# jeertmans/DiffeRT2d

Hardware: AMD Instinct MI355X
Metric: ray-path candidates/s (higher is better)
Workload: dtype f32

## Files before the change

### differt2d_amd/csrc/d2d_kernels.hpp

```cpp
#pragma once
#include <hip/hip_runtime.h>
#include <stdint.h>

#include "../../include/d2d.h"

namespace d2d {

template <typename T>
__device__ __forceinline__ const __attribute__((address_space(4))) T* cmem(const T* p) {
    return (const __attribute__((address_space(4))) T*)(unsigned long long)p;
}

__device__ __forceinline__ float4 ldc4(const float4* p, long i) {
    typedef float v4f __attribute__((ext_vector_type(4)));
    const v4f v = ((const __attribute__((address_space(4))) v4f*)(unsigned long long)p)[i];
    return make_float4(v.x, v.y, v.z, v.w);
}
__device__ __forceinline__ int4 ldc4i(const int4* p, long i) {
    typedef int v4i __attribute__((ext_vector_type(4)));
    const v4i v = ((const __attribute__((address_space(4))) v4i*)(unsigned long long)p)[i];
    return make_int4(v.x, v.y, v.z, v.w);
}

template <typename T, unsigned OFF>
__device__ __forceinline__ T late_kernarg() {
    static_assert(sizeof(T) == 4 || sizeof(T) == 8, "one or two dwords");
    const auto base = __builtin_amdgcn_kernarg_segment_ptr();
    T v;
    if constexpr (sizeof(T) == 8) asm volatile("s_load_dwordx2 %0, %1, %2\n\ts_waitcnt lgkmcnt(0)" : "=s"(v) : "s"(base), "i"(OFF));
    else asm volatile("s_load_dword %0, %1, %2\n\ts_waitcnt lgkmcnt(0)" : "=s"(v) : "s"(base), "i"(OFF));
    return v;
}
#define D2D_LATE_ARG(T, field) late_kernarg<T, (unsigned)__builtin_offsetof(SweepArgs, field)>()

enum Mode { MODE_HARD = 0, MODE_HSIG = 1, MODE_SIG = 2 };

constexpr int RL_CHUNK = 128;
struct ListPool {
    unsigned long long* pool;
    int* next;
    int* head;
    int n_static;
    int max_chunks;
};
struct RegionLevel {
    int* cnt[D2D_MAX_ORDER + 1];
    int chunk0[D2D_MAX_ORDER + 1];
    int S;
    int R;
    int regions_x, regions_y;
    const float4* box;
    const unsigned long long* hidden;
    float hidden_dperp;
};
struct RegionLists {
    RegionLevel leaf;
    ListPool lp;
    int* flag;
};

struct SweepArgs {
    const RegionLists* __restrict__ rl;
    int* fb_n;
    int* fb_list;
    const float4* __restrict__ occl;
    const float4* __restrict__ refl;
    const float4* __restrict__ flt;
    const int* __restrict__ cw;
    int N, Nc;
    const float* __restrict__ X;
    const float* __restrict__ Y;
    float* __restrict__ out;
    int m, n;
    float txx, txy;
    int min_order, max_order;
    float alpha, tol;
    float seg_lo, seg_hi;
    float flt_lo, flt_hi;
    float on_lo, on_hi;
    float loss_skip;
    float sig_l2f;
    int sig_mono;
    const unsigned long long* __restrict__ shadow;
    float shadow_dperp;
    float shadow_lo, shadow_inv;
    int shadow_prefix_ok;
    const unsigned long long* __restrict__ pair;
    float pair_dperp;
    int pair_prefix_ok;
    float fnum[D2D_MAX_ORDER + 1];
    float h2;
    int fun_id;
    int out_mode;
    float patch;
    float* __restrict__ grad;
    const float* __restrict__ cot;
    float* __restrict__ partial;
    const float* __restrict__ cust_f;
    const float* __restrict__ cust_pb;
    long cust_cells;

    const int* __restrict__ sched;
    int cullq_off;
    int n_heavy;
    int heavy_cap;
    float* __restrict__ heavy_list;
    int* __restrict__ heavy_cnt;
    int* __restrict__ heavy_done;
    unsigned* __restrict__ cost_out;

    unsigned long long* nan_cell_bits;
    unsigned* nan_row_bits;
    int nan_row_words;
    int nan_wqcap, nan_rb;
#ifdef D2D_AB_TIMELINE
    unsigned long long* tl_ring;
    int tl_seq;
#endif
    unsigned long long* stats;
    unsigned long long* wave_cycles;
};

#define D2D_WORK(x) (st.work += (x))
#define D2D_EPS 1.1920929e-07f

struct WaveStats {
    unsigned c[16];
    int shadow;
    unsigned work;
};

__device__ __forceinline__ bool wave_any(bool p) { return __any(p); }

__device__ __forceinline__ int late_index(int i) {
    asm volatile("" : "+s"(i));
    return i;
}

template <int I>
__device__ __forceinline__ void stat_add(WaveStats& st, unsigned long long x) {
    const unsigned x32 = (unsigned)x;
    asm volatile("v_add_u32 %0, %0, %1" : "+v"(st.c[I]) : "v"(x32));
}

#ifndef D2D_FAST_DIV
#define D2D_FAST_DIV 0
#endif
__device__ __forceinline__ bool div_in_range(float x) {
    float ax = fabsf(x);
    return ax >= 2.168404345e-19f && ax <= 4.611686018e18f;
}
__device__ __forceinline__ float rcp_refined(float y) {
    float r = __builtin_amdgcn_rcpf(y);
    float e = __builtin_fmaf(-y, r, 1.0f);
    return __builtin_fmaf(e, r, r);
}
__device__ __forceinline__ float div_with_rcp(float x, float y, float r) {
    float q = x * r;
    float e = __builtin_fmaf(-y, q, x);
    q = __builtin_fmaf(e, r, q);
    e = __builtin_fmaf(-y, q, x);
    return __builtin_fmaf(e, r, q);
}
__device__ __forceinline__ void div2_exact(float x1, float x2, float y, float& q1, float& q2) {
#if D2D_FAST_DIV
    const bool ok = div_in_range(y) && (x1 == 0.0f || div_in_range(x1)) && (x2 == 0.0f || div_in_range(x2));
    if (!wave_any(!ok)) {
        const float r = rcp_refined(y);
        q1 = div_with_rcp(x1, y, r);
        q2 = div_with_rcp(x2, y, r);
        return;
    }
#endif
    q1 = x1 / y;
    q2 = x2 / y;
}
__device__ __forceinline__ float div1_exact(float x, float y) {
#if D2D_FAST_DIV
    const bool ok = div_in_range(y) && (x == 0.0f || div_in_range(x));
    if (!wave_any(!ok)) return div_with_rcp(x, y, rcp_refined(y));
#endif
    return x / y;
}

__device__ __forceinline__ void image_of(const float4& r0, float px, float py, float& ox, float& oy) {
    float ix = px - r0.x, iy = py - r0.y;
    float dn = ix * r0.z + iy * r0.w;
    float s = 2.0f * dn;
    ox = px - s * r0.z;
    oy = py - s * r0.w;
}

__device__ __forceinline__ void normalize2(float vx, float vy, float& ox, float& oy) {
    float len = sqrtf(vx * vx + vy * vy);
    len = (len == 0.0f) ? 1.0f : len;
    ox = vx / len;
    oy = vy / len;
}

template <int B, int E, class F>
__device__ __forceinline__ void static_for(F&& f) {
    if constexpr (B < E) {
        f(std::integral_constant<int, B>{});
        static_for<B + 1, E>(f);
    }
}

__device__ __forceinline__ float clampact(float x, float alpha) {
    float z = alpha * x;
    return fminf(fmaxf(z + 3.0f, 0.0f), 6.0f);
}

static __device__ __constant__ unsigned long long EXPF_TAB[32] = {
    0x3ff0000000000000ull, 0x3fefd9b0d3158574ull, 0x3fefb5586cf9890full, 0x3fef9301d0125b51ull, 0x3fef72b83c7d517bull, 0x3fef54873168b9aaull,
    0x3fef387a6e756238ull, 0x3fef1e9df51fdee1ull, 0x3fef06fe0a31b715ull, 0x3feef1a7373aa9cbull, 0x3feedea64c123422ull, 0x3feece086061892dull,
    0x3feebfdad5362a27ull, 0x3feeb42b569d4f82ull, 0x3feeab07dd485429ull, 0x3feea47eb03a5585ull, 0x3feea09e667f3bcdull, 0x3fee9f75e8ec5f74ull,
    0x3feea11473eb0187ull, 0x3feea589994cce13ull, 0x3feeace5422aa0dbull, 0x3feeb737b0cdc5e5ull, 0x3feec49182a3f090ull, 0x3feed503b23e255dull,
    0x3feee89f995ad3adull, 0x3feeff76f2fb5e47ull, 0x3fef199bdd85529cull, 0x3fef3720dcef9069ull, 0x3fef5818dcfba487ull, 0x3fef7c97337b9b5full,
    0x3fefa4afa2a490daull, 0x3fefd0765b6e4540ull};
__device__ __forceinline__ float expf_libm(float x) {
    if (x != x) return x + x;
    if (x > 0x1.62e42ep6f) return __builtin_inff();
    if (x < -0x1.9fe368p6f) return 0.0f;
    if (x < -0x1.9d1d9ep6f) return 0x1p-149f;
    const double z = (0x1.71547652b82fep+0 * 32.0) * (double)x;
    double kd = z + 0x1.8p+52;
    const unsigned long long ki = (unsigned long long)__double_as_longlong(kd);
    kd = kd - 0x1.8p+52;
    const double r = z - kd;
    const unsigned long long t = EXPF_TAB[ki & 31ull] + (ki << 47);
    const double sc = __longlong_as_double((long long)t);
    const double zz = (0x1.c6af84b912394p-5 / 32.0 / 32.0 / 32.0) * r + (0x1.ebfce50fac4f3p-3 / 32.0 / 32.0);
    const double r2 = r * r;
    double y = (0x1.62e42ff0c52d6p-1 / 32.0) * r + 1.0;
    y = zz * r2 + y;
    y = y * sc;
    return (float)y;
}

__device__ __forceinline__ float sigmoidf_(float z) { return 1.0f / (1.0f + expf_libm(-z)); }

__device__ __forceinline__ float sig_zc_of(float l2f, float acc) {
    const int E = (int)((__float_as_uint(acc) >> 23) & 0xffu) - 127;
    return ((float)(E - 25) - l2f - 0.01f) * 0.69314718f;
}

struct GradCtx {
    float grx, gry;
    float tbx, tby;
    float cot;
    float* wl;
    bool scene;
    int ci;
    long cell;
};

__device__ __forceinline__ float wave_sum(float v) {
#pragma unroll
    for (int off = 32; off > 0; off >>= 1) v += __shfl_xor(v, off, 64);
    return v;
}

template <int MODE>
__device__ __forceinline__ float dact(float x, float alpha) {
    float z = alpha * x;
    if (MODE == MODE_HSIG) {
        float y = z + 3.0f;
        return (y > 0.0f && y < 6.0f) ? alpha / 6.0f : 0.0f;
    }
    float s = sigmoidf_(z);
    return alpha * (s * (1.0f - s));
}

__device__ __forceinline__ void normalize2_bwd(float vx, float vy, float obx, float oby, float& vbx, float& vby) {
    float len = sqrtf(vx * vx + vy * vy);
    bool z = (len == 0.0f);
    len = z ? 1.0f : len;
    float ox = vx / len, oy = vy / len;
    float d = z ? 0.0f : (obx * ox + oby * oy);
    vbx = (obx - d * ox) / len;
    vby = (oby - d * oy) / len;
}

template <int K, int MODE, bool STATS, bool GRAD = false, bool PREF = true, bool TXG = false>
__device__ __forceinline__ void eval_candidate(const SweepArgs& a, const int (&cand)[D2D_MAX_ORDER],
                                               const float (&imgx)[D2D_MAX_ORDER], const float (&imgy)[D2D_MAX_ORDER],
                                               float txx, float txy, float rxx, float rxy, bool lane_bad, float& acc,
                                               WaveStats& st, GradCtx* g = nullptr, float acc_floor = -1.0f) {
    const float zc_acc = (acc_floor >= 0.0f) ? acc_floor : acc;
    int on_i = 0, on_w = 0, hit_i = 0, hit_j = -1;
    float hit2 = -3.0e38f;
    bool znan = false;
    long cust = 0;
    if (GRAD && a.fun_id == D2D_FUN_CUSTOM) cust = (long)(g->ci++) * a.cust_cells + g->cell;
    float px[K + 2], py[K + 2];
    px[0] = txx;
    py[0] = txy;
    px[K + 1] = rxx;
    py[K + 1] = rxy;

    if (PREF && !GRAD && K > 0) {
        const float4 r0 = ldc4(a.refl, 2 * cand[K - 1]);
        const float4 r1 = ldc4(a.refl, 2 * cand[K - 1] + 1);
        const float4 fc = ldc4(a.flt, cand[K - 1]);
        float ux = rxx - imgx[K - 1], uy = rxy - imgy[K - 1];
        float vx = r0.x - rxx, vy = r0.y - rxy;
        float un = ux * r0.z + uy * r0.w;
        float vn = vx * r0.z + vy * r0.w;
        float gq = vn * __builtin_amdgcn_rcpf(un);
        float dx = __builtin_fmaf(gq, ux, -vx), dy = __builtin_fmaf(gq, uy, -vy);
        float sa = __builtin_fmaf(r1.y, dy, r1.x * dx) * fc.x;
        float ex = __builtin_fmaf(fabsf(gq), fabsf(ux), fabsf(vx)) + fabsf(r0.x);
        float ey = __builtin_fmaf(fabsf(gq), fabsf(uy), fabsf(vy)) + fabsf(r0.y);
        float M = __builtin_fmaf(__builtin_fmaf(fabsf(r1.y), ey, fabsf(r1.x) * ex), fc.y, 1e-30f);
        bool cull = !lane_bad && (un != 0.0f) && (ex < 1e18f) && (ey < 1e18f) && ((sa + M < a.on_lo) || (sa - M > a.on_hi));
        if (STATS) stat_add<9>(st, 1);
        if (!wave_any(!cull)) return;
    }

    D2D_WORK(6 + 2 * K);
    if (STATS) {
        stat_add<0>(st, 1);
        stat_add<6>(st, K);
    }
    float sv[K + 1];
    constexpr bool PRE = !GRAD && !TXG && K >= 1;
    unsigned long long sh_pre = 0ull, pm_pre[K + 1];
    constexpr bool HOIST = PRE && K <= 2;
    if (HOIST) {
        if (a.shadow != nullptr) sh_pre = cmem(a.shadow)[cand[0]];
#pragma unroll
        for (int i = 0; i + 1 < K; ++i) pm_pre[i] = (a.pair != nullptr) ? cmem(a.pair)[(size_t)cand[i] * a.N + cand[i + 1]] : 0ull;
    }
    const int sh = (st.shadow >= 0 && st.shadow < a.N) ? st.shadow : -1;
    int j = sh >= 0 ? sh : 0;
    float4 w = ldc4(a.occl, a.N > 0 ? j : 0);
    {
        float ptx = rxx, pty = rxy;
#pragma unroll
        for (int i = K - 1; i >= 0; --i) {
            const float4 r0 = ldc4(a.refl, 2 * cand[i]);
            float ux = ptx - imgx[i], uy = pty - imgy[i];
            float vx = r0.x - ptx, vy = r0.y - pty;
            float un = ux * r0.z + uy * r0.w;
            float vn = vx * r0.z + vy * r0.w;
            bool z = (un == 0.0f);
            float den = z ? 1.0f : un;
            float incx, incy;
            div2_exact(vn * ux, vn * uy, den, incx, incy);
            incx = z ? 0.0f : incx;
            incy = z ? 0.0f : incy;
            ptx = ptx + incx;
            pty = pty + incy;
            px[i + 1] = ptx;
            py[i + 1] = pty;
            if (GRAD && (MODE != MODE_HARD || a.fun_id != D2D_FUN_ONE)) znan = znan || z;
            if (!GRAD) {
                const float4 r1 = ldc4(a.refl, 2 * cand[i] + 1);
                const float dx = ptx - r0.x, dy = pty - r0.y;
                const float sw = div1_exact(r1.x * dx + r1.y * dy, r1.z);
                sv[i] = sw;
                if (i > 0) {
                    bool off;
                    if (MODE == MODE_HARD) off = !((sw >= 0.0f) && (sw <= 1.0f));
                    else if (MODE == MODE_HSIG) off = fminf(clampact(sw - 0.0f, a.alpha), clampact(1.0f - sw, a.alpha)) == 0.0f;
                    else off = fminf(a.alpha * (sw - 0.0f), a.alpha * (1.0f - sw)) <= fmaxf(-89.0f, sig_zc_of(a.sig_l2f, zc_acc));
                    const bool pt_bad = lane_bad || !(fabsf(ptx) < 1e18f) || !(fabsf(pty) < 1e18f);
                    if (!wave_any(!off || pt_bad)) {
                        if (STATS && i == K - 1) stat_add<15>(st, 1);
                        return;
                    }
                }
            }
        }
    }
    if (GRAD && MODE != MODE_HARD && K > 0) {
#pragma unroll
        for (int i = 0; i <= K; ++i) znan = znan || (px[i + 1] == px[i] && py[i + 1] == py[i]);
    }
    if (GRAD && a.fun_id != D2D_FUN_ONE && a.fun_id != D2D_FUN_CUSTOM) {
#pragma unroll
        for (int i = 0; i <= K; ++i) znan = znan || (((px[i + 1] - px[i]) + D2D_EPS == 0.0f) && ((py[i + 1] - py[i]) + D2D_EPS == 0.0f));
    }
    if (GRAD && wave_any(znan)) {
        const float qnan = __builtin_nanf("");
        if (znan) {
            g->grx = qnan;
            g->gry = qnan;
        }
        if (g->scene) {
            if (znan) g->tbx = g->tby = qnan;
            if ((threadIdx.x & 63) == 0) {
#pragma unroll
                for (int i = 0; i < K; ++i) {
                    float* w4 = g->wl + 4 * cand[i];
                    w4[0] = w4[1] = w4[2] = w4[3] = qnan;
                }
            }
        }
    }

    bool bad = lane_bad;
#pragma unroll
    for (int i = 1; i <= K; ++i) bad = bad || !(fabsf(px[i]) < 1e18f) || !(fabsf(py[i]) < 1e18f);
    if (GRAD && a.fun_id == D2D_FUN_CUSTOM) {
        const float* pb = a.cust_pb + cust * (2 * (D2D_MAX_ORDER + 2));
        bad = bad || !(fabsf(a.cust_f[cust]) < 3.0e38f);
#pragma unroll
        for (int i = 0; i < 2 * (K + 2); ++i) bad = bad || !(fabsf(pb[i]) < 3.0e38f);
    }

    bool on_b = true;
    float on_c = 6.0f;
    float on_z = 3.0e38f;
    bool nanflag = false;
#pragma unroll
    for (int i = 0; i < K; ++i) {
        float s;
        if (GRAD) {
            const float4 r0 = ldc4(a.refl, 2 * cand[i]);
            const float4 r1 = ldc4(a.refl, 2 * cand[i] + 1);
            float dx = px[i + 1] - r0.x, dy = py[i + 1] - r0.y;
            s = div1_exact(r1.x * dx + r1.y * dy, r1.z);
            sv[i] = s;
        } else {
            s = sv[i];
        }
        if (MODE == MODE_HARD) {
            on_b = on_b && (s >= 0.0f) && (s <= 1.0f);
        } else if (MODE == MODE_HSIG) {
            nanflag = nanflag || (s != s);
            float c1 = clampact(s - 0.0f, a.alpha), c2 = clampact(1.0f - s, a.alpha);
            float cm = fminf(c1, c2);
            if (GRAD && cm < on_c) {
                on_i = i;
                on_w = (c2 < c1) ? 1 : 0;
            }
            on_c = fminf(on_c, cm);
        } else {
            nanflag = nanflag || (s != s);
            float z1 = a.alpha * (s - 0.0f), z2 = a.alpha * (1.0f - s);
            float zm = fminf(z1, z2);
            if (GRAD && zm < on_z) {
                on_i = i;
                on_w = (z2 < z1) ? 1 : 0;
            }
            on_z = fminf(on_z, zm);
        }
    }
    bool on_zero = (MODE == MODE_HARD) ? !on_b : (MODE == MODE_HSIG) ? (on_c == 0.0f)
                   : (on_z <= (GRAD ? -89.0f : fmaxf(-89.0f, sig_zc_of(a.sig_l2f, zc_acc))));
    if (K > 0 && !wave_any(!on_zero || bad)) return;

    const bool live = !on_zero || bad;
    D2D_WORK(1);

    float bx[K + 1], by[K + 1];
#pragma unroll
    for (int i = 0; i <= K; ++i) {
        bx[i] = px[i] - px[i + 1];
        by[i] = py[i] - py[i + 1];
    }
    bool hit_b = false;
    float hit_c = 0.0f;
    float hit_z = -3.0e38f;
    bool any_test = false;
    bool active = live;
    if (!GRAD && !TXG && K >= 1 && a.shadow != nullptr) {
        const float eps = 1.1920929e-07f;
        bool occl = false;
        float Ei[K + 1];
        float padv[K + 1];
#pragma unroll
        for (int i = 0; i < K; ++i) {
            const float4 r0 = ldc4(a.refl, 2 * cand[i]);
            const float4 r1 = ldc4(a.refl, 2 * cand[i] + 1);
            const float4 fc = ldc4(a.flt, cand[i]);
            const float ex = fabsf(px[i + 1] - px[i + 2]) + fabsf(r0.x - px[i + 2]) + fabsf(r0.x) + fabsf(imgx[i]);
            const float ey = fabsf(py[i + 1] - py[i + 2]) + fabsf(r0.y - py[i + 2]) + fabsf(r0.y) + fabsf(imgy[i]);
            Ei[i] = ex + ey;
            padv[i] = __builtin_fmaf(__builtin_fmaf(fabsf(r1.y), ey, fabsf(r1.x) * ex), fc.y, 1e-4f);
        }
        {
            const unsigned long long shm = HOIST ? sh_pre : cmem(a.shadow)[cand[0]];
            if (shm != 0ull) {
                const float fa_ = (sv[0] - padv[0] - a.shadow_lo) * a.shadow_inv, fb_ = (sv[0] + padv[0] - a.shadow_lo) * a.shadow_inv;
                const bool ok = fa_ >= 0.0f && fb_ < 64.0f && 256.0f * eps * Ei[0] <= a.shadow_dperp;
                const int ka = ok ? (int)fa_ : 0, kb = ok ? (int)fb_ : 0;
                occl = ok && (kb - ka <= 1) && ((shm >> ka) & 1ull) && ((shm >> kb) & 1ull);
            }
        }
        if (K >= 2 && a.pair != nullptr) {
#pragma unroll
            for (int i = 0; i + 1 < K; ++i) {
                const unsigned long long m = HOIST ? pm_pre[i] : cmem(a.pair)[(size_t)cand[i] * a.N + cand[i + 1]];
                if (m != 0ull) {
                    const float k8 = 0.125f * a.shadow_inv;
                    const float ea_ = (sv[i] - padv[i] - a.shadow_lo) * k8, eb_ = (sv[i] + padv[i] - a.shadow_lo) * k8;
                    const float la_ = (sv[i + 1] - padv[i + 1] - a.shadow_lo) * k8, lb_ = (sv[i + 1] + padv[i + 1] - a.shadow_lo) * k8;
                    const bool ok = ea_ >= 0.0f && eb_ < 8.0f && la_ >= 0.0f && lb_ < 8.0f && 512.0f * eps * Ei[i] <= a.pair_dperp &&
                                    512.0f * eps * Ei[i + 1] <= a.pair_dperp;
                    const int ea = ok ? (int)ea_ : 0, eb = ok ? (int)eb_ : 0, la = ok ? (int)la_ : 0, lb = ok ? (int)lb_ : 0;
                    const bool all4 = ((m >> (ea + 8 * la)) & 1ull) && ((m >> (eb + 8 * la)) & 1ull) && ((m >> (ea + 8 * lb)) & 1ull) &&
                                      ((m >> (eb + 8 * lb)) & 1ull);
                    occl = occl || (ok && all4 && (eb - ea <= 1) && (lb - la <= 1));
                }
            }
        }
        if (wave_any(occl)) {
            if (MODE == MODE_HARD) hit_b = hit_b || occl;
            else if (MODE == MODE_HSIG) hit_c = occl ? 6.0f : hit_c;
            else {
                hit_z = occl ? 1.0e30f : hit_z;
                any_test = true;
            }
            active = active && (!occl || bad);
            D2D_WORK(2);
            if (!wave_any(active)) return;
        }
    }
    if (STATS) stat_add<2>(st, 1);
    constexpr bool PAIRS = MODE != MODE_SIG;
    if constexpr (PAIRS) {
    auto filt = [&](const float4& ww, int jj) -> unsigned {
        unsigned wbits = 0u;
#pragma unroll
        for (int i = 0; i <= K; ++i) {
            const int ig0 = (i == 0) ? -1 : cand[i - 1];
            const int ig1 = (i == K) ? -1 : cand[i];
            const bool skip = (jj == ig0 || jj == ig1);
            float Cx = ww.x - px[i], Cy = ww.y - py[i];
            float fa = by[i] * Cx - bx[i] * Cy;
            float fb = ww.z * Cy - ww.w * Cx;
            float fd = ww.w * bx[i] - ww.z * by[i];
            float pa = __builtin_fmaf(-a.flt_lo, fd, fa) * __builtin_fmaf(-a.flt_hi, fd, fa);
            float pb = __builtin_fmaf(-a.flt_lo, fd, fb) * __builtin_fmaf(-a.flt_hi, fd, fb);
            bool miss = fmaxf(pa, pb) > 0.0f;
            if (MODE == MODE_SIG && !skip) any_test = true;
            if (STATS) stat_add<4>(st, skip ? 0 : 1);
            wbits |= (!skip && active && (!miss || bad)) ? (1u << i) : 0u;
        }
        return wbits;
    };
    auto exact = [&](const float4& ww, int jj, unsigned wbits) {
#pragma unroll
        for (int i = 0; i <= K; ++i) {
            if (!wave_any((wbits >> i) & 1u)) continue;
            if (STATS) stat_add<5>(st, 1);
            D2D_WORK(2);
            const float Cx = ww.x - px[i], Cy = ww.y - py[i];
            const float fa = by[i] * Cx - bx[i] * Cy;
            const float fb = ww.z * Cy - ww.w * Cx;
            const float fd = ww.w * bx[i] - ww.z * by[i];
            bool dz = (fd == 0.0f);
            float dd = dz ? 1.0f : fd;
            float ta, tb;
            div2_exact(fa, fb, dd, ta, tb);
            ta = dz ? __builtin_inff() : ta;
            tb = dz ? __builtin_inff() : tb;
            if (MODE == MODE_HARD) {
                bool h = (ta >= a.seg_lo) && (ta <= a.seg_hi) && (tb >= a.seg_lo) && (tb <= a.seg_hi);
                hit_b = hit_b || h;
            } else if (MODE == MODE_HSIG) {
                nanflag = nanflag || (ta != ta) || (tb != tb);
                float c = fminf(fminf(clampact(ta - a.seg_lo, a.alpha), clampact(a.seg_hi - ta, a.alpha)),
                                fminf(clampact(tb - a.seg_lo, a.alpha), clampact(a.seg_hi - tb, a.alpha)));
                if (GRAD && (c > hit_c || (c == hit_c && hit_j >= 0 && (jj < hit_j || (jj == hit_j && i < hit_i))))) {
                    hit_i = i;
                    hit_j = jj;
                }
                if (GRAD) hit2 = (c > hit_c) ? hit_c : fmaxf(hit2, c);
                hit_c = fmaxf(hit_c, c);
            } else {
                nanflag = nanflag || (ta != ta) || (tb != tb);
                float z = fminf(fminf(a.alpha * (ta - a.seg_lo), a.alpha * (a.seg_hi - ta)),
                                fminf(a.alpha * (tb - a.seg_lo), a.alpha * (a.seg_hi - tb)));
                if (GRAD && (z > hit_z || (z == hit_z && hit_j >= 0 && (jj < hit_j || (jj == hit_j && i < hit_i))))) {
                    hit_i = i;
                    hit_j = jj;
                }
                if (GRAD) hit2 = (z > hit_z) ? hit_z : fmaxf(hit2, z);
                hit_z = fmaxf(hit_z, z);
            }
        }
        if (MODE == MODE_HARD) active = active && (!hit_b || bad);
        else if (MODE == MODE_HSIG) active = active && (hit_c != 6.0f || bad);
        else active = active && (hit_z < 17.5f || bad);
    };
    {
        bool done = a.N <= 0;
        if (!done && sh >= 0) {
            const unsigned b0 = filt(w, sh);
            D2D_WORK(K + 1);
            if (wave_any(b0 != 0u)) {
                exact(w, sh, b0);
                if (!wave_any(active)) {
                    st.shadow = sh;
                    done = true;
                }
            }
        }
        auto next_idx = [&](int x) -> int {
            ++x;
            return x == sh ? x + 1 : x;
        };
        int jA = (sh == 0) ? 1 : 0;
        if (!done && jA < a.N) {
            int jB = next_idx(jA);
            float4 wA = (sh >= 0) ? ldc4(a.occl, jA) : w;
            float4 wB = ldc4(a.occl, jB < a.N ? jB : jA);
            while (true) {
                const bool hasB = jB < a.N;
                const int nA = next_idx(jB), nB = next_idx(nA);
                const float4 wnA = ldc4(a.occl, nA < a.N ? nA : jA), wnB = ldc4(a.occl, nB < a.N ? nB : jA);
                const unsigned ba = filt(wA, jA);
                const unsigned bb = hasB ? filt(wB, jB) : 0u;
                D2D_WORK(hasB ? 2 * (K + 1) : (K + 1));
                if (wave_any((ba | bb) != 0u)) {
                    if (wave_any(ba != 0u)) {
                        exact(wA, jA, ba);
                        if (!wave_any(active)) {
                            st.shadow = jA;
                            break;
                        }
                    }
                    if (wave_any(bb != 0u)) {
                        exact(wB, jB, bb);
                        if (!wave_any(active)) {
                            st.shadow = jB;
                            break;
                        }
                    }
                }
                if (!(nA < a.N)) break;
                jA = nA;
                jB = nB;
                wA = wnA;
                wB = wnB;
            }
        }
    }
    } else {
    int nxt = sh >= 0 ? 0 : 1;
    if (nxt == sh) ++nxt;
    for (bool more = a.N > 0; more;) {
        const bool has_next = nxt < a.N;
        const float4 wn = ldc4(a.occl, has_next ? nxt : j);
        float fa_[K + 1], fb_[K + 1], fd_[K + 1];
        unsigned wbits = 0u;
#pragma unroll
        for (int i = 0; i <= K; ++i) {
            const int ig0 = (i == 0) ? -1 : cand[i - 1];
            const int ig1 = (i == K) ? -1 : cand[i];
            const bool skip = (j == ig0 || j == ig1);
            float Cx = w.x - px[i], Cy = w.y - py[i];
            float fa = by[i] * Cx - bx[i] * Cy;
            float fb = w.z * Cy - w.w * Cx;
            float fd = w.w * bx[i] - w.z * by[i];
            float pa = __builtin_fmaf(-a.flt_lo, fd, fa) * __builtin_fmaf(-a.flt_hi, fd, fa);
            float pb = __builtin_fmaf(-a.flt_lo, fd, fb) * __builtin_fmaf(-a.flt_hi, fd, fb);
            bool miss = fmaxf(pa, pb) > 0.0f;
            if (MODE == MODE_SIG && !skip) any_test = true;
            if (STATS) stat_add<4>(st, skip ? 0 : 1);
            wbits |= (!skip && active && (!miss || bad)) ? (1u << i) : 0u;
            fa_[i] = fa;
            fb_[i] = fb;
            fd_[i] = fd;
        }
        D2D_WORK(K + 1);
        if (wave_any(wbits != 0u)) {
#pragma unroll
            for (int i = 0; i <= K; ++i) {
                if (!wave_any((wbits >> i) & 1u)) continue;
                if (STATS) stat_add<5>(st, 1);
                D2D_WORK(2);
                const float fa = fa_[i], fb = fb_[i], fd = fd_[i];
                bool dz = (fd == 0.0f);
                float dd = dz ? 1.0f : fd;
                float ta, tb;
                div2_exact(fa, fb, dd, ta, tb);
                ta = dz ? __builtin_inff() : ta;
                tb = dz ? __builtin_inff() : tb;
                if (MODE == MODE_HARD) {
                    bool h = (ta >= a.seg_lo) && (ta <= a.seg_hi) && (tb >= a.seg_lo) && (tb <= a.seg_hi);
                    hit_b = hit_b || h;
                } else if (MODE == MODE_HSIG) {
                    nanflag = nanflag || (ta != ta) || (tb != tb);
                    float c = fminf(fminf(clampact(ta - a.seg_lo, a.alpha), clampact(a.seg_hi - ta, a.alpha)),
                                    fminf(clampact(tb - a.seg_lo, a.alpha), clampact(a.seg_hi - tb, a.alpha)));
                    if (GRAD && (c > hit_c || (c == hit_c && hit_j >= 0 && (j < hit_j || (j == hit_j && i < hit_i))))) {
                        hit_i = i;
                        hit_j = j;
                    }
                    if (GRAD) hit2 = (c > hit_c) ? hit_c : fmaxf(hit2, c);
                    hit_c = fmaxf(hit_c, c);
                } else {
                    nanflag = nanflag || (ta != ta) || (tb != tb);
                    float z = fminf(fminf(a.alpha * (ta - a.seg_lo), a.alpha * (a.seg_hi - ta)),
                                    fminf(a.alpha * (tb - a.seg_lo), a.alpha * (a.seg_hi - tb)));
                    if (GRAD && (z > hit_z || (z == hit_z && hit_j >= 0 && (j < hit_j || (j == hit_j && i < hit_i))))) {
                        hit_i = i;
                        hit_j = j;
                    }
                    if (GRAD) hit2 = (z > hit_z) ? hit_z : fmaxf(hit2, z);
                    hit_z = fmaxf(hit_z, z);
                }
            }
            if (MODE == MODE_HARD) active = active && (!hit_b || bad);
            else if (MODE == MODE_HSIG) active = active && (hit_c != 6.0f || bad);
            else active = active && (hit_z < 17.5f || bad);
            if (!wave_any(active)) {
                st.shadow = j;
                break;
            }
        }
        more = has_next;
        j = nxt;
        w = wn;
        ++nxt;
        if (nxt == sh) ++nxt;
    }
    }
    if (!wave_any(active)) return;

    if (STATS) stat_add<1>(st, 1);
    D2D_WORK(4 * K);
    float loss = 0.0f;
    bool loss_known = (K == 0);
    if (K > 0) {
        const float c = 8e-6f;
        float nvx[K + 1], nvy[K + 1];
#pragma unroll
        for (int i = 0; i <= K; ++i) {
            float vx = px[i + 1] - px[i], vy = py[i + 1] - py[i];
            float inv = __builtin_amdgcn_rsqf(__builtin_fmaf(vx, vx, vy * vy));
            nvx[i] = vx * inv;
            nvy[i] = vy * inv;
        }
        float bound = 0.0f;
#pragma unroll
        for (int i = 0; i < K; ++i) {
            const float4 r0 = ldc4(a.refl, 2 * late_index(cand[i]));
            float s2 = 2.0f * __builtin_fmaf(nvx[i], r0.z, nvy[i] * r0.w);
            float ex = __builtin_fmaf(s2, r0.z, nvx[i + 1] - nvx[i]);
            float ey = __builtin_fmaf(s2, r0.w, nvy[i + 1] - nvy[i]);
            bound += __builtin_fmaf(2.0f * c, fabsf(ex) + fabsf(ey), __builtin_fmaf(ex, ex, ey * ey)) + c * c;
        }
        const bool certain = (bound * 1.00001f < a.loss_skip) && !bad;
        loss_known = !wave_any(!certain && active);
    }
    if (!loss_known) {
#pragma unroll
        for (int i = 0; i < K; ++i) {
            const float4 r0 = ldc4(a.refl, 2 * late_index(cand[i]));
            float ix, iy, rx_, ry_;
            normalize2(px[i + 1] - px[i], py[i + 1] - py[i], ix, iy);
            normalize2(px[i + 2] - px[i + 1], py[i + 2] - py[i + 1], rx_, ry_);
            float din = ix * r0.z + iy * r0.w;
            float s2 = 2.0f * din;
            float ex = rx_ - (ix - s2 * r0.z);
            float ey = ry_ - (iy - s2 * r0.w);
            loss = loss + (ex * ex + ey * ey);
        }
        if (STATS) stat_add<7>(st, K);
    }
    bool ok_b = loss < a.tol;
    float ok_x = a.tol - loss;
    if (MODE != MODE_HARD) nanflag = nanflag || (loss != loss);

    float valid;
    float on_v = 1.0f, nh_v = 1.0f, ok_v = 1.0f;
    if (MODE == MODE_HARD) {
        valid = (on_b && !hit_b && ok_b) ? 1.0f : 0.0f;
    } else if (MODE == MODE_HSIG) {
        on_v = on_c / 6.0f;
        float hit_v = hit_c / 6.0f;
        ok_v = clampact(ok_x, a.alpha) / 6.0f;
        nh_v = 1.0f - hit_v;
        valid = fminf(fminf(on_v, nh_v), ok_v);
        valid = nanflag ? 0.0f : valid;
    } else {
        on_v = (K == 0) ? 1.0f : sigmoidf_(on_z);
        float hit_v = any_test ? fmaxf(0.0f, sigmoidf_(hit_z)) : 0.0f;
        ok_v = sigmoidf_(a.alpha * ok_x);
        nh_v = 1.0f - hit_v;
        valid = fminf(fminf(on_v, nh_v), ok_v);
        valid = nanflag ? 0.0f : valid;
    }

    if (!wave_any(valid != 0.0f || bad)) return;
    if (STATS) stat_add<3>(st, 1), stat_add<8>(st, K + 1);
    D2D_WORK(6);
    float r = 0.0f;
#pragma unroll
    for (int i = 0; i <= K; ++i) {
        float vx = (px[i + 1] - px[i]) + D2D_EPS;
        float vy = (py[i + 1] - py[i]) + D2D_EPS;
        r = r + sqrtf(vx * vx + vy * vy);
    }
    float f;
    if (a.fun_id == D2D_FUN_RECEIVED_POWER) f = a.fnum[K] / (a.h2 + r * r);
    else if (a.fun_id == D2D_FUN_LENGTH_SQUARED) f = r * r;
    else if (a.fun_id == D2D_FUN_LENGTH) f = r;
    else if (GRAD && a.fun_id == D2D_FUN_CUSTOM) f = a.cust_f[cust];
    else f = 1.0f;
    acc = acc + valid * f;

    if (GRAD) {
        const float fbar = valid;
        const float vbar = (MODE == MODE_HARD || nanflag) ? 0.0f : f;
        float rbar;
        if (a.fun_id == D2D_FUN_RECEIVED_POWER) {
            float Dn = a.h2 + r * r;
            rbar = -(fbar * (f / Dn)) * (2.0f * r);
        } else if (a.fun_id == D2D_FUN_LENGTH_SQUARED) rbar = fbar * (2.0f * r);
        else if (a.fun_id == D2D_FUN_LENGTH) rbar = fbar;
        else rbar = 0.0f;

        float pbx[K + 2], pby[K + 2];
#pragma unroll
        for (int i = 0; i < K + 2; ++i) pbx[i] = pby[i] = 0.0f;
        if (a.fun_id == D2D_FUN_CUSTOM) {
            const float* pb = a.cust_pb + cust * (2 * (D2D_MAX_ORDER + 2));
#pragma unroll
            for (int i = 0; i < K + 2; ++i) {
                pbx[i] = fbar * pb[2 * i];
                pby[i] = fbar * pb[2 * i + 1];
            }
        }
        if (a.fun_id != D2D_FUN_ONE && a.fun_id != D2D_FUN_CUSTOM) {
#pragma unroll
            for (int i = 0; i <= K; ++i) {
                float wx = (px[i + 1] - px[i]) + D2D_EPS, wy = (py[i + 1] - py[i]) + D2D_EPS;
                float len = sqrtf(wx * wx + wy * wy);
                float gx = rbar * (wx / len), gy = rbar * (wy / len);
                pbx[i + 1] += gx; pby[i + 1] += gy;
                pbx[i] -= gx; pby[i] -= gy;
            }
        }
        constexpr int KK = (K > 0) ? K : 1;
        float obx[KK], oby[KK], nbx[KK], nby[KK], tbx[KK], tby[KK];
#pragma unroll
        for (int i = 0; i < KK; ++i) obx[i] = oby[i] = nbx[i] = nby[i] = tbx[i] = tby[i] = 0.0f;
        float p1bx = 0.0f, p1by = 0.0f, abx = 0.0f, aby = 0.0f;
        bool occ = false;

        if (MODE != MODE_HARD) {
            float w_on = (on_v < nh_v) ? 1.0f : (nh_v < on_v) ? 0.0f : 0.5f;
            float w_nh = 1.0f - w_on, w_ok = 0.0f;
            {
                const float m01 = fminf(on_v, nh_v);
                const float keep = (m01 < ok_v) ? 1.0f : (ok_v < m01) ? 0.0f : 0.5f;
                w_on *= keep;
                w_nh *= keep;
                w_ok = 1.0f - keep;
            }
            const float vb_on = vbar * w_on, vb_nh = vbar * w_nh, vb_ok = vbar * w_ok;
            float lossbar = (w_ok != 0.0f) ? -(vb_ok * dact<MODE>(ok_x, a.alpha)) : 0.0f;
            if (K > 0 && wave_any(lossbar != 0.0f)) {
#pragma unroll
                for (int i = 0; i < K; ++i) {
                    const float4 r0 = ldc4(a.refl, 2 * cand[i]);
                    float v1x = px[i + 1] - px[i], v1y = py[i + 1] - py[i];
                    float v2x = px[i + 2] - px[i + 1], v2y = py[i + 2] - py[i + 1];
                    float ix, iy, rx_, ry_;
                    normalize2(v1x, v1y, ix, iy);
                    normalize2(v2x, v2y, rx_, ry_);
                    float din = ix * r0.z + iy * r0.w;
                    float s2 = 2.0f * din;
                    float ex = rx_ - (ix - s2 * r0.z), ey = ry_ - (iy - s2 * r0.w);
                    float ebx = 2.0f * ex * lossbar, eby = 2.0f * ey * lossbar;
                    float rbx = ebx, rby = eby;
                    float ibx = -ebx, iby = -eby;
                    float s2b = ebx * r0.z + eby * r0.w;
                    nbx[i] += s2 * ebx; nby[i] += s2 * eby;
                    float dinb = 2.0f * s2b;
                    ibx += dinb * r0.z; iby += dinb * r0.w;
                    nbx[i] += dinb * ix; nby[i] += dinb * iy;
                    float a1x, a1y, a2x, a2y;
                    normalize2_bwd(v1x, v1y, ibx, iby, a1x, a1y);
                    normalize2_bwd(v2x, v2y, rbx, rby, a2x, a2y);
                    pbx[i + 1] += a1x; pby[i + 1] += a1y; pbx[i] -= a1x; pby[i] -= a1y;
                    pbx[i + 2] += a2x; pby[i + 2] += a2y; pbx[i + 1] -= a2x; pby[i + 1] -= a2y;
                }
            }
            if (K > 0) {
#pragma unroll
                for (int i = 0; i < K; ++i) {
                    const float4 r0 = ldc4(a.refl, 2 * cand[i]);
                    const float4 r1 = ldc4(a.refl, 2 * cand[i] + 1);
                    float dx = px[i + 1] - r0.x, dy = py[i + 1] - r0.y;
                    float s = (r1.x * dx + r1.y * dy) / r1.z;
                    float x = on_w ? (1.0f - s) : (s - 0.0f);
                    float sb = (w_on != 0.0f && i == on_i) ? vb_on * dact<MODE>(x, a.alpha) * (on_w ? -1.0f : 1.0f) : 0.0f;
                    float q = sb / r1.z;
                    pbx[i + 1] += q * r1.x; pby[i + 1] += q * r1.y;
                    obx[i] -= q * r1.x; oby[i] -= q * r1.y;
                    bool degenerate = (r1.x * r1.x + r1.y * r1.y == 0.0f);
                    float sqb = degenerate ? 0.0f : -(q * s);
                    tbx[i] += q * dx + 2.0f * sqb * r1.x;
                    tby[i] += q * dy + 2.0f * sqb * r1.y;
                }
            }
            occ = (w_nh != 0.0f) && (hit_j >= 0) && (vb_nh != 0.0f);
            auto occluder_adjoint = [&](auto ic, const float4& w, float wgt, float& o_p1bx, float& o_p1by, float& o_abx, float& o_aby) {
                constexpr int i = decltype(ic)::value;
                const float qx = px[i], qy = py[i], q1x = px[i + 1], q1y = py[i + 1];
                float Bx = qx - q1x, By = qy - q1y;
                float Cx = w.x - qx, Cy = w.y - qy;
                float fa = By * Cx - Bx * Cy, fb = w.z * Cy - w.w * Cx, fd = w.w * Bx - w.z * By;
                bool dz = (fd == 0.0f);
                float dd = dz ? 1.0f : fd;
                float ta = dz ? __builtin_inff() : fa / dd, tb = dz ? __builtin_inff() : fb / dd;
                float x0 = ta - a.seg_lo, x1 = a.seg_hi - ta, x2 = tb - a.seg_lo, x3 = a.seg_hi - tb;
                float m0, m1, m2, m3;
                if (MODE == MODE_HSIG) { m0 = clampact(x0, a.alpha); m1 = clampact(x1, a.alpha); m2 = clampact(x2, a.alpha); m3 = clampact(x3, a.alpha); }
                else { m0 = a.alpha * x0; m1 = a.alpha * x1; m2 = a.alpha * x2; m3 = a.alpha * x3; }
                if (MODE == MODE_SIG) { m0 = sigmoidf_(m0); m1 = sigmoidf_(m1); m2 = sigmoidf_(m2); m3 = sigmoidf_(m3); }
                const float a0 = (m0 < m1) ? 1.0f : (m1 < m0) ? 0.0f : 0.5f, b0 = (m2 < m3) ? 1.0f : (m3 < m2) ? 0.0f : 0.5f;
                const float mA = fminf(m0, m1), mB = fminf(m2, m3);
                const float ab = (mA < mB) ? 1.0f : (mB < mA) ? 0.0f : 0.5f;
                const float k0 = ab * a0, k1 = ab * (1.0f - a0), k2 = (1.0f - ab) * b0, k3 = (1.0f - ab) * (1.0f - b0);
                const float hw = (wgt != 0.0f && !dz) ? -(vb_nh * wgt) : 0.0f;
                const float h0 = (k0 != 0.0f) ? hw * k0 * dact<MODE>(x0, a.alpha) : 0.0f, h1 = (k1 != 0.0f) ? hw * k1 * dact<MODE>(x1, a.alpha) : 0.0f;
                const float h2 = (k2 != 0.0f) ? hw * k2 * dact<MODE>(x2, a.alpha) : 0.0f, h3 = (k3 != 0.0f) ? hw * k3 * dact<MODE>(x3, a.alpha) : 0.0f;
                float tab = h0 - h1, tbb = h2 - h3;
                float fab = tab / dd, fbb = tbb / dd;
                float fdb = -(tab * ta + tbb * tb) / dd;
                fdb = (tab != 0.0f || tbb != 0.0f) ? fdb : 0.0f;
                float Bbx = -fab * Cy + fdb * w.w, Bby = fab * Cx - fdb * w.z;
                float Cbx = fab * By - fbb * w.w, Cby = -fab * Bx + fbb * w.z;
                o_abx = fbb * Cy - fdb * By;
                o_aby = -fbb * Cx + fdb * Bx;
                o_p1bx = Cbx; o_p1by = Cby;
                pbx[i] += Bbx - Cbx; pby[i] += Bby - Cby;
                pbx[i + 1] -= Bbx; pby[i + 1] -= Bby;
            };
            bool tie = false;
            float vmax = 0.0f;
            if (wave_any(occ)) {
                if (MODE == MODE_HSIG) {
                    vmax = hit_c;
// ... 3023 lines not shown
```

Measured before the change: 28320 billion.

## Add wave-level interval bounding-box prefilter to skip occluder walls in batches

For low-order non-gradient paths, each wave computes a bounding box of all active lanes' path vertices using DPP min/max reductions. It then runs an interval-arithmetic test per 64-wall chunk, one wall per lane, to drop walls that cannot intersect any lane's path segments. Only the surviving walls, taken from a ballot mask, go through the existing per-wall filter and exact test. This removes most per-wall work when paths are spatially coherent. It costs an extra reduction and interval test per chunk and uses inline DPP assembly, which is fragile.

```diff
diff --git a/differt2d_amd/csrc/d2d_kernels.hpp b/differt2d_amd/csrc/d2d_kernels.hpp
--- a/differt2d_amd/csrc/d2d_kernels.hpp
+++ b/differt2d_amd/csrc/d2d_kernels.hpp
@@ -3,6 +3,7 @@
 #include <stdint.h>
 
 #include "../../include/d2d.h"
+#include "d2d_wallfilter.hpp"
 
 namespace d2d {
 
@@ -261,6 +262,23 @@
     return v;
 }
 
+#define D2D_BOX_STEP(c)                                          \
+    "v_min_f32_dpp %0, %0, %0 " c " row_mask:0xf bank_mask:0xf\n\t" \
+    "v_max_f32_dpp %1, %1, %1 " c " row_mask:0xf bank_mask:0xf\n\t" \
+    "v_min_f32_dpp %2, %2, %2 " c " row_mask:0xf bank_mask:0xf\n\t" \
+    "v_max_f32_dpp %3, %3, %3 " c " row_mask:0xf bank_mask:0xf\n\t"
+__device__ __forceinline__ void wave_box(float& x0, float& x1, float& y0, float& y1) {
+    asm volatile("s_nop 1\n\t" D2D_BOX_STEP("row_shr:1") D2D_BOX_STEP("row_shr:2") D2D_BOX_STEP("row_shr:4") D2D_BOX_STEP("row_shr:8")
+                     D2D_BOX_STEP("row_bcast:15") D2D_BOX_STEP("row_bcast:31") "s_nop 0"
+                 : "+v"(x0), "+v"(x1), "+v"(y0), "+v"(y1));
+    auto last = [](float v) { return __int_as_float(__builtin_amdgcn_readlane(__float_as_int(v), 63)); };
+    x0 = last(x0);
+    x1 = last(x1);
+    y0 = last(y0);
+    y1 = last(y1);
+}
+#undef D2D_BOX_STEP
+
 template <int MODE>
 __device__ __forceinline__ float dact(float x, float alpha) {
     float z = alpha * x;
@@ -600,6 +618,91 @@
                 }
             }
         }
+        if constexpr (!GRAD && K <= 2) {
+        const int lane = threadIdx.x & 63;
+        bool pre = !done && !wave_any(bad) && wf_window_ok(a.flt_lo, a.flt_hi) && __ballot(1) == ~0ull;
+        auto bundle = [&](WfSeg (&S)[K + 1]) -> bool {
+            constexpr int U = TXG ? K + 1 : 0;
+            const float inf = __builtin_inff();
+            WfBox P[K + 2];
+            bool ok = true;
+#pragma unroll
+            for (int i = 0; i <= K + 1; ++i) {
+                if (i == U) {
+                    P[i] = WfBox{px[i], px[i], py[i], py[i]};
+                } else {
+                    P[i] = WfBox{active ? px[i] : inf, active ? px[i] : -inf, active ? py[i] : inf, active ? py[i] : -inf};
+                    wave_box(P[i].x0, P[i].x1, P[i].y0, P[i].y1);
+                }
+                ok = ok && wf_box_ok(P[i]);
+            }
+            auto uni = [](float v) { return __int_as_float(__builtin_amdgcn_readfirstlane(__float_as_int(v))); };
+#pragma unroll
+            for (int i = 0; i <= K; ++i) {
+                const WfSeg t = wf_segment(P[i], P[i + 1]);
+                S[i] = WfSeg{P[i], uni(t.bx0), uni(t.bx1), uni(t.by0), uni(t.by1)};
+            }
+            D2D_WORK(K + 1);
+            return ok;
+        };
+        auto pop = [](unsigned long long& mm, int base) -> int {
+            if (mm == 0ull) return -1;
+            const int b = __builtin_ctzll(mm);
+            mm &= mm - 1ull;
+            return base + b;
+        };
+        for (int base = 0; base < a.N && !done; base += 64) {
+            const int nin = a.N - base;
+            unsigned long long m = nin >= 64 ? ~0ull : (1ull << nin) - 1ull;
+            if (pre) {
+                const float4 row = a.occl[min(base + lane, a.N - 1)];
+                WfSeg S[K + 1];
+                pre = bundle(S);
+                if (pre) {
+                    const bool clear = wf_wall_clear<K>(S, cand, base + lane, row.x, row.y, row.z, row.w, a.flt_lo, a.flt_hi);
+                    m &= ~__ballot(clear);
+                    D2D_WORK(3 * (K + 1));
+                    if (STATS) stat_add<9>(st, (K + 2) / 2);
+                }
+            }
+            if (sh >= base && sh < base + 64) m &= ~(1ull << (sh - base));
+            int jA = pop(m, base), jB = pop(m, base);
+            if (jA < 0) continue;
+            float4 wA = ldc4(a.occl, jA);
+            float4 wB = ldc4(a.occl, jB >= 0 ? jB : jA);
+            while (true) {
+                const bool hasB = jB >= 0;
+                const int nA = pop(m, base), nB = pop(m, base);
+                const float4 wnA = ldc4(a.occl, nA >= 0 ? nA : jA), wnB = ldc4(a.occl, nB >= 0 ? nB : jA);
+                const unsigned ba = filt(wA, jA);
+                const unsigned bb = hasB ? filt(wB, jB) : 0u;
+                D2D_WORK(hasB ? 2 * (K + 1) : (K + 1));
+                if (wave_any((ba | bb) != 0u)) {
+                    if (wave_any(ba != 0u)) {
+                        exact(wA, jA, ba);
+                        if (!wave_any(active)) {
+                            st.shadow = jA;
+                            done = true;
+                            break;
+                        }
+                    }
+                    if (wave_any(bb != 0u)) {
+                        exact(wB, jB, bb);
+                        if (!wave_any(active)) {
+                            st.shadow = jB;
+                            done = true;
+                            break;
+                        }
+                    }
+                }
+                if (nA < 0) break;
+                jA = nA;
+                jB = nB;
+                wA = wnA;
+                wB = wnB;
+            }
+        }
+        } else {
         auto next_idx = [&](int x) -> int {
             ++x;
             return x == sh ? x + 1 : x;
@@ -638,6 +741,7 @@
                 wA = wnA;
                 wB = wnB;
             }
+        }
         }
     }
     } else {
diff --git a/differt2d_amd/csrc/d2d_wallfilter.hpp b/differt2d_amd/csrc/d2d_wallfilter.hpp
--- /dev/null
+++ b/differt2d_amd/csrc/d2d_wallfilter.hpp
@@ -0,0 +1,84 @@
+#pragma once
+
+#if defined(__HIPCC__) || defined(__CUDACC__)
+#define D2D_WF_HD __host__ __device__ __forceinline__
+#else
+#include <math.h>
+#define D2D_WF_HD inline
+#endif
+
+namespace d2d {
+
+constexpr float WF_TINY = 1e-18f;
+constexpr float WF_BIG = 1e18f;
+constexpr float WF_WIN = 16.0f;
+
+struct WfBox {
+    float x0, x1, y0, y1;
+};
+
+D2D_WF_HD bool wf_window_ok(float flt_lo, float flt_hi) { return flt_lo <= 0.0f && flt_lo >= -WF_WIN && flt_hi >= 0.0f && flt_hi <= WF_WIN; }
+D2D_WF_HD bool wf_box_ok(const WfBox& b) {
+    return fmaxf(fmaxf(fabsf(b.x0), fabsf(b.x1)), fmaxf(fabsf(b.y0), fabsf(b.y1))) < WF_BIG && b.x0 <= b.x1 && b.y0 <= b.y1;
+}
+
+D2D_WF_HD void wf_mul(float u0, float u1, float v0, float v1, float& lo, float& hi) {
+    const float a = u0 * v0, b = u0 * v1, c = u1 * v0, d = u1 * v1;
+    lo = fminf(fminf(a, b), fminf(c, d));
+    hi = fmaxf(fmaxf(a, b), fmaxf(c, d));
+}
+D2D_WF_HD void wf_scale(float s, float v0, float v1, float& lo, float& hi) {
+    const float a = s * v0, b = s * v1;
+    lo = fminf(a, b);
+    hi = fmaxf(a, b);
+}
+
+struct WfSeg {
+    WfBox p;
+    float bx0, bx1, by0, by1;
+};
+D2D_WF_HD WfSeg wf_segment(const WfBox& p, const WfBox& q) {
+    return WfSeg{p, p.x0 - q.x1, p.x1 - q.x0, p.y0 - q.y1, p.y1 - q.y0};
+}
+
+D2D_WF_HD bool wf_segment_clear(const WfSeg& s, float wx, float wy, float wz, float ww, float flt_lo, float flt_hi) {
+    const float cx0 = wx - s.p.x1, cx1 = wx - s.p.x0;
+    const float cy0 = wy - s.p.y1, cy1 = wy - s.p.y0;
+    float u0, u1, v0, v1;
+    wf_mul(s.by0, s.by1, cx0, cx1, u0, u1);
+    wf_mul(s.bx0, s.bx1, cy0, cy1, v0, v1);
+    const float fa0 = u0 - v1, fa1 = u1 - v0;
+    wf_scale(wz, cy0, cy1, u0, u1);
+    wf_scale(ww, cx0, cx1, v0, v1);
+    const float fb0 = u0 - v1, fb1 = u1 - v0;
+    wf_scale(ww, s.bx0, s.bx1, u0, u1);
+    wf_scale(wz, s.by0, s.by1, v0, v1);
+    const float fd0 = u0 - v1, fd1 = u1 - v0;
+    const float nl = -flt_lo, nh = -flt_hi;
+    const float al0 = __builtin_fmaf(nl, fd0, fa0), al1 = __builtin_fmaf(nl, fd1, fa1);
+    const float ah0 = __builtin_fmaf(nh, fd1, fa0), ah1 = __builtin_fmaf(nh, fd0, fa1);
+    const float bl0 = __builtin_fmaf(nl, fd0, fb0), bl1 = __builtin_fmaf(nl, fd1, fb1);
+    const float bh0 = __builtin_fmaf(nh, fd1, fb0), bh1 = __builtin_fmaf(nh, fd0, fb1);
+    const bool pa = (fminf(al0, ah0) >= WF_TINY) | (fmaxf(al1, ah1) <= -WF_TINY);
+    const bool pb = (fminf(bl0, bh0) >= WF_TINY) | (fmaxf(bl1, bh1) <= -WF_TINY);
+    return pa | pb;
+}
+
+template <int K, int NC>
+D2D_WF_HD bool wf_wall_clear(const WfSeg (&S)[K + 1], const int (&cand)[NC], int j, float wx, float wy, float wz, float ww, float flt_lo,
+                             float flt_hi) {
+    bool clear = fmaxf(fmaxf(fabsf(wx), fabsf(wy)), fmaxf(fabsf(wz), fabsf(ww))) < WF_BIG;
+#if defined(__HIP_DEVICE_COMPILE__)
+#pragma unroll
+#endif
+    for (int i = 0; i <= K; ++i) {
+        const int ig0 = (i == 0) ? -1 : cand[i - 1];
+        const int ig1 = (i == K) ? -1 : cand[i];
+        const bool joins = (j == ig0) | (j == ig1);
+        const bool seg = wf_segment_clear(S[i], wx, wy, wz, ww, flt_lo, flt_hi);
+        clear = clear & (joins | seg);
+    }
+    return clear;
+}
+
+}
```

Result: faster. 33330 billion, median of 6 (+17.7%).
